# passcod/zarc

Hardware: AMD Instinct MI355X
Metric: uncompressed GiB/s (pack) at zstd -3 (higher is better)
Workload: dtype u8; 1 GPU; zarc pack 10000 x 1048576 B synthetic entries per GPU, zstd level 3, checksum on (BASELINE configs[1]); entries_per_gpu=10000, entries_total=10000, entry_bytes=1048576, level=3, kinds=text/records/lz/random round-robin

## Files before the change

zarc_amd/csrc/zarc_device.h:

```cpp
#pragma once
#include <hip/hip_runtime.h>
#include <stdint.h>

namespace zd {

constexpr int WAVE = 64;

__device__ __forceinline__ int lane_id() { return (int)(threadIdx.x & 63); }
__device__ __forceinline__ int wave_id() { return (int)(threadIdx.x >> 6); }

__device__ __forceinline__ void wave_sync()
{
#ifdef ZARC_HIPEMU
    hipemu_wave_sync();
#else
    __builtin_amdgcn_fence(__ATOMIC_RELEASE, "wavefront");
    __builtin_amdgcn_wave_barrier();
    __builtin_amdgcn_fence(__ATOMIC_ACQUIRE, "wavefront");
#endif
}

__device__ __forceinline__ void wave_lds_order()
{
#ifdef ZARC_HIPEMU
    hipemu_wave_sync();
#else
    asm volatile("" ::: "memory");
#endif
}

__device__ __forceinline__ void lds_barrier()
{
#ifdef ZARC_HIPEMU
    __syncthreads();
#else
    asm volatile("s_waitcnt lgkmcnt(0)\n\ts_barrier" ::: "memory");
#endif
}

template <int PRIO> __device__ __forceinline__ void wave_priority()
{
#ifndef ZARC_HIPEMU
    __builtin_amdgcn_s_setprio(PRIO);
#endif
}

__device__ __forceinline__ void wave_sync_global()
{
#ifdef ZARC_HIPEMU
    hipemu_wave_sync();
#else
    __builtin_amdgcn_fence(__ATOMIC_RELEASE, "workgroup");
    __builtin_amdgcn_wave_barrier();
    __builtin_amdgcn_fence(__ATOMIC_ACQUIRE, "workgroup");
#endif
}

__device__ __forceinline__ uint32_t uniform(uint32_t v)
{
#ifdef ZARC_HIPEMU
    return hipemu_readfirstlane(v);
#else
    return (uint32_t)__builtin_amdgcn_readfirstlane((int)v);
#endif
}

__device__ __forceinline__ uint32_t readlane(uint32_t v, uint32_t idx)
{
#ifdef ZARC_HIPEMU
    return hipemu_readfirstlane((uint32_t)__shfl((int)v, (int)idx, 64));
#else
    return (uint32_t)__builtin_amdgcn_readlane((int)v, (int)__builtin_amdgcn_readfirstlane((int)idx));
#endif
}

__device__ __forceinline__ uint64_t ballot(bool p) { return (uint64_t)__ballot(p ? 1 : 0); }
__device__ __forceinline__ uint32_t shfl(uint32_t v, int src) { return (uint32_t)__shfl((int)v, src, 64); }
__device__ __forceinline__ uint32_t shfl_up(uint32_t v, unsigned d) { return (uint32_t)__shfl_up((int)v, d, 64); }
__device__ __forceinline__ uint32_t shfl_down(uint32_t v, unsigned d) { return (uint32_t)__shfl_down((int)v, d, 64); }
__device__ __forceinline__ uint32_t shfl_xor(uint32_t v, int m) { return (uint32_t)__shfl_xor((int)v, m, 64); }

__device__ __forceinline__ uint32_t load_l2_u32(const uint32_t *p)
{
#ifdef ZARC_HIPEMU
    return *p;
#else
    return __hip_atomic_load(p, __ATOMIC_RELAXED, __HIP_MEMORY_SCOPE_AGENT);
#endif
}
__device__ __forceinline__ uint64_t load_l2_u64(const uint32_t *p)
{
#ifdef ZARC_HIPEMU
    return (uint64_t)p[0] | ((uint64_t)p[1] << 32);
#else
    return __hip_atomic_load((const uint64_t *)p, __ATOMIC_RELAXED, __HIP_MEMORY_SCOPE_AGENT);
#endif
}
__device__ __forceinline__ void atomic_max_l2(uint32_t *p, uint32_t v)
{
#ifdef ZARC_HIPEMU
    if (*p < v) *p = v;
#else
    (void)__hip_atomic_fetch_max(p, v, __ATOMIC_RELAXED, __HIP_MEMORY_SCOPE_AGENT);
#endif
}
__device__ __forceinline__ void wait_vmem()
{
#ifndef ZARC_HIPEMU
    asm volatile("s_waitcnt vmcnt(0)" ::: "memory");
#endif
}

__device__ __forceinline__ void store_streaming(uint64_t *p, uint64_t v)
{
#ifdef ZARC_HIPEMU
    *p = v;
#else
    __builtin_nontemporal_store(v, p);
#endif
}

__device__ __forceinline__ uint32_t rotr32(uint32_t x, int n) { return (x >> n) | (x << (32 - n)); }
__device__ __forceinline__ uint64_t rotl64(uint64_t x, int n) { return (x << n) | (x >> (64 - n)); }
__device__ __forceinline__ int hb32(uint32_t v) { return 31 - __clz((int)v); }
__device__ __forceinline__ int ctz64(uint64_t v) { return __ffsll((long long)v) - 1; }
__device__ __forceinline__ int ctz32(uint32_t v) { return __ffs((int)v) - 1; }

__device__ __forceinline__ uint32_t wave_scan_incl(uint32_t v)
{
#ifdef ZARC_HIPEMU
    int l = lane_id();
#pragma unroll
    for (int d = 1; d < 64; d <<= 1) {
        uint32_t t = shfl_up(v, (unsigned)d);
        if (l >= d) v += t;
    }
    return v;
#else
    v += (uint32_t)__builtin_amdgcn_update_dpp(0, (int)v, 0x111, 0xF, 0xF, false);
    v += (uint32_t)__builtin_amdgcn_update_dpp(0, (int)v, 0x112, 0xF, 0xF, false);
    v += (uint32_t)__builtin_amdgcn_update_dpp(0, (int)v, 0x114, 0xF, 0xF, false);
    v += (uint32_t)__builtin_amdgcn_update_dpp(0, (int)v, 0x118, 0xF, 0xF, false);
    v += (uint32_t)__builtin_amdgcn_update_dpp(0, (int)v, 0x142, 0xA, 0xF, false);
    v += (uint32_t)__builtin_amdgcn_update_dpp(0, (int)v, 0x143, 0xC, 0xF, false);
    return v;
#endif
}
__device__ __forceinline__ uint32_t shfl_up1(uint32_t v)
{
#ifdef ZARC_HIPEMU
    return shfl_up(v, 1u);
#else
    return (uint32_t)__builtin_amdgcn_update_dpp((int)v, (int)v, 0x138, 0xF, 0xF, false);
#endif
}
__device__ __forceinline__ uint32_t row_scan_incl(uint32_t v)
{
#ifdef ZARC_HIPEMU
    int l = lane_id() & 15;
#pragma unroll
    for (int d = 1; d < 16; d <<= 1) {
        uint32_t t = shfl_up(v, (unsigned)d);
        if (l >= d) v += t;
    }
    return v;
#else
    v += (uint32_t)__builtin_amdgcn_update_dpp(0, (int)v, 0x111, 0xF, 0xF, false);
    v += (uint32_t)__builtin_amdgcn_update_dpp(0, (int)v, 0x112, 0xF, 0xF, false);
    v += (uint32_t)__builtin_amdgcn_update_dpp(0, (int)v, 0x114, 0xF, 0xF, false);
    v += (uint32_t)__builtin_amdgcn_update_dpp(0, (int)v, 0x118, 0xF, 0xF, false);
    return v;
#endif
}
__device__ __forceinline__ uint32_t wave_sum(uint32_t v)
{
#pragma unroll
    for (int d = 32; d > 0; d >>= 1) v += shfl_xor(v, d);
    return v;
}
__device__ __forceinline__ uint32_t wave_max(uint32_t v)
{
#pragma unroll
    for (int d = 32; d > 0; d >>= 1) { uint32_t t = shfl_xor(v, d); v = t > v ? t : v; }
    return v;
}

__device__ __forceinline__ uint32_t load_u32(const uint8_t *p)
{
    uint32_t v;
    __builtin_memcpy(&v, p, 4);
    return v;
}
__device__ __forceinline__ uint64_t load_u64(const uint8_t *p)
{
    uint64_t v;
    __builtin_memcpy(&v, p, 8);
    return v;
}

}
```

zarc_amd/csrc/zge_match.hip:

```cpp
#include "zarc_device.h"
#include "zarc_kernels.h"

namespace {

#ifdef ZARC_HIPEMU
#define ZGE_CLOCK() 0ull
#else
#define ZGE_CLOCK() ((unsigned long long)__builtin_readcyclecounter())
#endif
#define ZGE_IDX(u) ((uint32_t)((wave * PER + (u)) * 64 + lane))
#ifndef ZGE_S2_DUPMASK
#define ZGE_S2_DUPMASK 0
#endif
#define ZGE_PROF(i) do { if ((dbg & 1024) && tid == 0) { const unsigned long long now_ = ZGE_CLOCK(); L.prof[i] += now_ - tprev; tprev = now_; } } while (0)

constexpr int TILE = 1024;
constexpr int THREADS = 512;
constexpr int WAVES = THREADS / 64;
constexpr int PER = TILE / THREADS;
static_assert(PER == 2, "the kernel is written for two positions per thread");
constexpr int CHUNKS = TILE / 64;
constexpr int TAG_BITS = 10;
constexpr uint32_t TAG_MASK = (1u << TAG_BITS) - 1;
struct U128 { uint64_t lo, hi; };
constexpr int CAP_MAX = 256;
constexpr int REP_BACK_MAX = 256;
constexpr int TB_BYTES = 12 + REP_BACK_MAX + TILE + CAP_MAX + 24;

template <int TAB_LOG, bool NEAR16> struct MatchLds {
    static constexpr int TAB_WORDS = NEAR16 ? (1 << TAB_LOG) / 2 : 2 << TAB_LOG;
    uint32_t tab[TAB_WORDS + (NEAR16 ? 1 : 0)];
    uint32_t a0[TILE], a1[TILE];
    uint32_t ex[TILE];
    uint32_t tb[2][(TB_BYTES + 3) / 4];
    uint32_t wcnt[CHUNKS];
    uint32_t wrep[2 * CHUNKS];
    uint32_t ctrl[16];
    unsigned long long prof[15];
};
enum { K_POS = 0, K_REP0 = 1, K_REP1 = 2, K_FLAG = 3, K_SLOT = 4, K_ANY = 5, K_CHG = 6 ,
       K_CEND = 10 ,
       K_CLEN = 11 ,
       K_LONG = 12 , K_LONG2 = 13  };

__device__ __forceinline__ uint32_t hash_long32(uint64_t v)
{
    const uint32_t lo = (uint32_t)v, hi = (uint32_t)(v >> 32);
    return lo * 0x9E3779B1u + hi * 0x85EBCA77u;
}
__device__ __forceinline__ uint32_t hash_far32(uint64_t v, uint32_t w) { return hash_long32(v) + w * 0xC2B2AE3Du; }
__device__ __forceinline__ uint32_t hash_short32(uint64_t v, int nbytes)
{
    uint32_t lo = (uint32_t)v, hi = (uint32_t)(v >> 32);
    if (nbytes < 8) hi &= (nbytes > 4) ? ((1u << (8 * (nbytes - 4))) - 1) : 0u;
    if (nbytes < 4) lo &= (1u << (8 * nbytes)) - 1;
    return lo * 0xC2B2AE3Du + hi * 0x27D4EB2Fu;
}

constexpr int REP_COST = 9;
constexpr int F_REP_BACK = 256, F_BACK_CAP = 8, F_LAZY_DELTA = 5, F_MIN_REP = 3, F_SEG_LOG = 21;
template <int MATCH_COST, int LITC> __device__ __forceinline__ int32_t score_mc(uint32_t len, uint32_t off, bool is_rep)
{
    static_assert(LITC == 5 || LITC == 6, "literal cost");
    const int32_t lits = (int32_t)((len << 2) + (LITC == 6 ? len << 1 : len));
    return is_rep ? lits - REP_COST : lits - MATCH_COST - zd::hb32(off);
}
#define score_of(P_, len_, off_, rep_) score_mc<MATCH_COST, LITC>((len_), (off_), (rep_))

template <bool WIDE> __device__ __forceinline__ uint32_t match_pack_w(uint32_t off, uint32_t len, bool rep) { return off | (len << 21) | ((rep ? 1u : 0u) << (WIDE ? 31 : 30)); }
__device__ __forceinline__ uint32_t match_off(uint32_t m) { return m & 0x1FFFFFu; }
template <bool WIDE> __device__ __forceinline__ uint32_t match_len_w(uint32_t m) { return (m >> 21) & (WIDE ? 0x3FFu : 0x1FFu); }
template <bool WIDE> __device__ __forceinline__ bool match_rep_w(uint32_t m) { return WIDE ? (m >> 31) != 0 : ((m >> 30) & 1u) != 0; }
#define match_pack(o_, l_, r_) match_pack_w<(CONT_CAP > 0 || EXT_ROUND)>((o_), (l_), (r_))
#define match_len(m_) match_len_w<(CONT_CAP > 0 || EXT_ROUND)>(m_)
#define match_rep(m_) match_rep_w<(CONT_CAP > 0 || EXT_ROUND)>(m_)
constexpr int LONG_CAP = 960;

__device__ __forceinline__ uint32_t wave_match_ext(const uint8_t *src, uint32_t p, uint32_t off, uint32_t from, uint32_t maxlen, int lane)
{
    static_assert(LONG_CAP <= 1024, "one trip of 64 x 16 bytes");
    const uint32_t at = from + 16u * (uint32_t)lane;
    const bool act = at < maxlen;
    U128 a{0, 0}, b{0, 0};
    if (act) { __builtin_memcpy(&a, src + (p + at), 16); __builtin_memcpy(&b, src + (p - off + at), 16); }
    const uint64_t xl = a.lo ^ b.lo, xh = a.hi ^ b.hi;
    const uint32_t mis = xl ? (uint32_t)(zd::ctz64(xl) >> 3) : (xh ? 8u + (uint32_t)(zd::ctz64(xh) >> 3) : 16u);
    const uint64_t bad = zd::ballot(act && mis < 16u);
    uint32_t len = maxlen;
    if (bad) {
        const uint32_t first = (uint32_t)zd::ctz64(bad);
        len = from + 16u * first + zd::readlane(mis, first);
        if (len > maxlen) len = maxlen;
    }
    return len;
}

struct StageWin { const uint32_t *w; int ndw; uint32_t wofs; };
static_assert((TB_BYTES + 3) / 4 <= THREADS, "one staged dword per thread");
__device__ __forceinline__ StageWin stage_window(const ZgeParams &P, const uint8_t *src, uint32_t n, uint32_t tile, uint32_t tend, uint32_t cap_max)
{
    (void)P;
    const uint32_t before = (uint32_t)F_REP_BACK + 8;
    const uint32_t lo = tile >= before ? tile - before : 0;
    uint32_t hi = tend + cap_max + 16;
    if (hi > n + 16) hi = n + 16;
    const uintptr_t a = (uintptr_t)(src + lo);
    const uint32_t mis = (uint32_t)(a & 3);
    StageWin s;
    s.w = (const uint32_t *)(a - mis);
    s.ndw = (int)((hi - lo + mis + 3) / 4);
    s.wofs = mis - lo;
    return s;
}

__device__ __forceinline__ uint32_t tile_end(uint32_t tile, uint32_t n)
{
    uint32_t e = tile + TILE;
    const uint32_t be = (tile / ZARC_BLOCK + 1) * ZARC_BLOCK;
    if (e > be) e = be;
    return e > n ? n : e;
}

}

template <int TAB_LOG, int SHORT_BYTES, int MATCH_COST, int F_FAR_LOG, int FAR_WAYS, bool FAR_SHORT, int FAR_STEP_LOG, int FAR_RES_LOG, int FAR_SKIP, int FAR_BACK, bool DIAG,
          bool NEAR16, int FAR_CDC, int LITC, int LAZY2, bool REP_PASS, int CONT_CAP, bool EXT_ROUND>
__device__ __forceinline__ void zge_match_body(MatchLds<TAB_LOG, NEAR16> &L, const ZgeParams &P, const uint8_t *__restrict__ src_base, const uint64_t *__restrict__ src_off,
                                               const uint64_t *__restrict__ src_len, const uint32_t *__restrict__ order, const uint32_t *__restrict__ units, uint32_t n_units,
                                               const uint64_t *__restrict__ block_prefix, ZgeBlock *__restrict__ blocks,
                                               uint64_t *__restrict__ seq_scratch, uint8_t *__restrict__ lit_scratch, uint32_t *__restrict__ queue,
                                               uint32_t *__restrict__ far_scratch)
{
    constexpr int NFAR = FAR_WAYS * (FAR_SHORT ? 2 : 1);
    constexpr int NTAB = 1 + NFAR;
    constexpr int far_shift = 32 - (F_FAR_LOG + TAG_BITS);
    constexpr uint32_t far_words = (uint32_t)(((size_t)FAR_WAYS << F_FAR_LOG) * (FAR_SHORT ? 2 : 1));
    uint32_t *const far_l = far_scratch + (size_t)blockIdx.x * far_words;
    uint32_t *const far_s = far_l + ((size_t)FAR_WAYS << F_FAR_LOG);
    constexpr uint32_t far_smask = (1u << FAR_STEP_LOG) - 1, far_rmask = (1u << FAR_RES_LOG) - 1;
    static_assert(FAR_BACK % 8 == 0 && FAR_BACK >= 8 && FAR_BACK <= 48, "backward extension of far candidates");
    static_assert(!FAR_CDC || (FAR_WAYS == 1 && !FAR_SHORT && far_shift >= FAR_CDC), "content-defined sampling: one way on the 12-byte hash");
    constexpr uint32_t cdc_mask = (1u << FAR_CDC) - 1;
    uint32_t *const Ltl = L.tab, *const Lts = L.tab + (NEAR16 ? 0 : (1 << TAB_LOG));
    typedef uint16_t __attribute__((may_alias)) u16a;
    u16a *const Lt16 = (u16a *)L.tab;
    const int tid = (int)threadIdx.x, lane = zd::lane_id();
    const uint32_t dbg = DIAG ? (uint32_t)P.dbg : 0u;
    const int wave = (int)zd::uniform((uint32_t)zd::wave_id());
    const uint64_t lt = (1ull << lane) - 1;
    const uint32_t seg_mask = (1u << F_SEG_LOG) - 1;
    const uint32_t cap_max = (uint32_t)(P.cap < CAP_MAX ? P.cap : CAP_MAX);
    unsigned long long tprev = ZGE_CLOCK();
    if (tid < 15) L.prof[tid] = 0;

    constexpr uint32_t SEG_BLOCKS = (1u << F_SEG_LOG) / ZARC_BLOCK;
    for (;;) {
    if (tid == 0) L.ctrl[K_SLOT] = atomicAdd(queue, 1u);
    zd::lds_barrier();
    const uint32_t unit = L.ctrl[K_SLOT];
    if (unit >= n_units) break;
    const uint32_t slot = units[2 * unit], ub0 = units[2 * unit + 1];
    const uint32_t f = order[slot];
    const uint8_t *src = src_base + src_off[f];
    const uint32_t n = (uint32_t)src_len[f];
    const uint32_t window = n <= (1u << P.window_log) ? (n ? n : 1u) : (1u << P.window_log);
    const uint32_t hash_end = n >= 8 ? n - 7 : 0;
    const bool far_on = NFAR && n > (uint32_t)P.far_min_frame;
    const uint32_t far_end = (far_on && n >= 12) ? n - 11 : 0;
    const uint64_t first_block = block_prefix[slot];
    const uint32_t nblocks = (uint32_t)(block_prefix[slot + 1] - first_block);

    for (int i = tid; i < MatchLds<TAB_LOG, NEAR16>::TAB_WORDS; i += THREADS) L.tab[i] = 0;
    if (NFAR && far_on) {
        uint4 *f4 = (uint4 *)far_l;
        for (uint32_t i = (uint32_t)tid; i < far_words / 4; i += THREADS) f4[i] = make_uint4(0, 0, 0, 0);
        zd::wait_vmem();
    }
    if (tid == 0) { L.ctrl[K_REP0] = 0; L.ctrl[K_REP1] = 0; }
    zd::lds_barrier();
    uint32_t cold = 0, skip_left = 0;
    constexpr bool FAR_COMPACT = FAR_RES_LOG > 0 && !FAR_CDC;
    constexpr int FNEXT_ROWS = FAR_COMPACT ? 1 : PER;
    uint32_t fnext[FNEXT_ROWS][NFAR ? NFAR : 1];
    uint32_t pf_far_tile = 0xFFFFFFFFu;
    uint32_t hfn[PER] = {0xFFFFFFFFu, 0xFFFFFFFFu};
    uint32_t pf_word = 0, pf_tile = 0xFFFFFFFFu;
    uint32_t lds_tile[2] = {0xFFFFFFFFu, 0xFFFFFFFFu};
#pragma unroll
    for (int u = 0; u < FNEXT_ROWS; u++)
#pragma unroll
        for (int k = 0; k < (NFAR ? NFAR : 1); k++) fnext[u][k] = 0;

    const uint32_t ub1 = (n > ZARC_SPLIT_MIN && ub0 + SEG_BLOCKS < nblocks) ? ub0 + SEG_BLOCKS : nblocks;
    for (uint32_t b = ub0; b < ub1; b++) {
        const uint32_t bs = b * ZARC_BLOCK;
        const uint32_t be = n - bs > ZARC_BLOCK ? bs + ZARC_BLOCK : n;
        const uint32_t blen = (uint32_t)(be - bs);
        ZgeBlock *rec = blocks + first_block + b;
        uint64_t *seq_out = seq_scratch + (first_block + b) * zge_seq_stride((uint32_t)P.slot_bytes);
        uint8_t *lit_out = lit_scratch + (first_block + b) * zge_lit_stride((uint32_t)P.slot_bytes);

        if (b > ub0 && (bs & seg_mask) == 0) {
            for (int i = tid; i < MatchLds<TAB_LOG, NEAR16>::TAB_WORDS; i += THREADS) L.tab[i] = 0;
            if (NFAR) {
                uint4 *f4 = (uint4 *)far_l;
                for (uint32_t i = (uint32_t)tid; i < far_words / 4; i += THREADS) f4[i] = make_uint4(0, 0, 0, 0);
                zd::wait_vmem();
                pf_far_tile = 0xFFFFFFFFu;
            }
        }
        if (tid == 0) { L.ctrl[K_FLAG] = 0; L.ctrl[K_POS] = 0; if (CONT_CAP) L.ctrl[K_CEND] = 0xFFFFFFFFu; }
        zd::lds_barrier();
        const uint8_t first = blen ? src[bs] : 0;
        const uint64_t pat = 0x0101010101010101ull * first;
        const uint64_t *w = (const uint64_t *)(src + bs);
        if (blen >= 1024 && tid < 128 && w[tid] != pat) L.ctrl[K_FLAG] = 1;
        zd::lds_barrier();
        if (L.ctrl[K_FLAG] == 0) {
            bool diff = false;
            const uint32_t nw = blen / 8;
            for (uint32_t i = (uint32_t)tid; i < nw; i += THREADS) diff |= w[i] != pat;
            for (uint32_t i = nw * 8 + (uint32_t)tid; i < blen; i += THREADS) diff |= src[bs + i] != first;
            if (diff) L.ctrl[K_FLAG] = 1;
        }
        zd::lds_barrier();
        const bool all_same = L.ctrl[K_FLAG] == 0;
        if (tid == 0) {
            rec->frame = f; rec->index = b; rec->src_len = blen; rec->nseq = 0; rec->nlit = 0;
            rec->type = (all_same && blen >= 2) ? 1u : 2u; rec->out_len = 0; rec->pad = 0;
        }
        if (all_same && blen >= 2) { zd::lds_barrier(); continue; }

        uint32_t nseq = 0, lp = 0;

        for (uint32_t tile = bs; tile < be; tile += TILE) {
            const uint32_t tend = be - tile > TILE ? tile + TILE : be;
            const uint32_t tcount = (uint32_t)(tend - tile);
            const uint32_t segbase = tile & ~seg_mask;
            zd::lds_barrier();
            ZGE_PROF(0);
            const uint32_t pos = bs + L.ctrl[K_POS];
            const bool cont = CONT_CAP && L.ctrl[K_CEND] == L.ctrl[K_POS] && pos >= tile;
            if (pos >= tend) { if (NFAR) zd::wait_vmem(); continue; }
            if (skip_left) {
                skip_left--;
                const uint32_t start = (uint32_t)((pos > tile ? pos : tile) - tile);
                {
                    const uint32_t cntb = tcount - start, k = (uint32_t)tid * 16;
                    const uint8_t *sp = src + tile + start;
                    uint8_t *dp = lit_out + lp;
                    if (!(dbg & 32)) {
                        if (k + 16 <= cntb) { U128 v; __builtin_memcpy(&v, sp + k, 16); __builtin_memcpy(dp + k, &v, 16); }
                        else for (uint32_t r = k; r < cntb; r++) dp[r] = sp[r];
                    }
                }
                lp += tcount - start;
                if (NFAR) zd::wait_vmem();
                zd::lds_barrier();
                if (tid == 0) L.ctrl[K_POS] = (uint32_t)(tend - bs);
                continue;
            }
            const uint32_t erep0 = L.ctrl[K_REP0], erep1 = L.ctrl[K_REP1];
            if (CONT_CAP && cont) {
                const uint32_t idx_c = pos - tile;
                if (wave == (int)(idx_c >> 7)) {
                    const uint32_t limit = (uint32_t)(be - pos);
                    uint32_t clen = 0;
                    if (erep0 != 0 && erep0 <= pos && erep0 <= window) clen = wave_match_ext(src, pos, erep0, 0, limit < (uint32_t)CONT_CAP ? limit : (uint32_t)CONT_CAP, lane);
                    if (lane == 0) L.ctrl[K_CLEN] = clen;
                }
            }
            if (tid == 0) L.ctrl[K_ANY] = 0;
            if (REP_PASS && tid < 4) L.ctrl[K_CHG + tid] = 0;
            if (EXT_ROUND && tid == 0) { L.ctrl[K_LONG] = 0; L.ctrl[K_LONG2] = 0; }

            const uint32_t bsel = (tile / TILE) & 1u;
            const uint8_t *const tbb = (const uint8_t *)L.tb[bsel];
            const uint8_t *const tbn = (const uint8_t *)L.tb[bsel ^ 1u];
            const StageWin sw = stage_window(P, src, n, tile, tend, cap_max);
            const uint32_t wofs = sw.wofs;
            const uint32_t ntile = tile + TILE;
            uint32_t wofs_n = 0;
            bool staged_now = false;
            {
                if (lds_tile[bsel] != tile) {
                    uint32_t v = pf_word;
                    if (pf_tile != tile && tid < sw.ndw) v = sw.w[tid];
                    if (tid < sw.ndw) L.tb[bsel][tid] = v;
                    lds_tile[bsel] = tile;
                    staged_now = true;
                }
                if (ntile < n) {
                    const StageWin nw = stage_window(P, src, n, ntile, tile_end(ntile, n), cap_max);
                    wofs_n = nw.wofs;
                    uint32_t v = pf_word;
                    if (pf_tile != ntile && tid < nw.ndw) v = nw.w[tid];
                    if (tid < nw.ndw) L.tb[bsel ^ 1u][tid] = v;
                    lds_tile[bsel ^ 1u] = ntile;
                    const uint32_t n2 = ntile + TILE;
                    if (n2 < n) {
                        const StageWin w2 = stage_window(P, src, n, n2, tile_end(n2, n), cap_max);
                        if (tid < w2.ndw) pf_word = w2.w[tid];
                        pf_tile = n2;
                    }
                }
            }
            if (staged_now) zd::lds_barrier();
            ZGE_PROF(1);
            uint64_t p8[PER];
            uint32_t fe[PER][NFAR ? NFAR : 1], ftag[PER][FAR_SHORT ? 2 : 1];
            uint32_t foffs[PER][NFAR ? NFAR : 1];
            uint64_t qf[PER][NFAR ? NFAR : 1];
            const bool far_ahead = NFAR && pf_far_tile == tile;
#pragma unroll
            for (int u = 0; u < PER; u++) {
                const uint32_t idx = ZGE_IDX(u);
                const uint32_t p = tile + idx;
                uint32_t hl = 0xFFFFFFFFu, hs = 0xFFFFFFFFu;
                p8[u] = 0;
#pragma unroll
                for (int k = 0; k < (NFAR ? NFAR : 1); k++) {
                    if (FAR_COMPACT) {
                        const uint32_t got = zd::shfl(fnext[0][k], (int)(((uint32_t)u * 64u + (uint32_t)lane) >> FAR_RES_LOG));
                        fe[u][k] = (far_ahead && !(idx & far_rmask)) ? got : 0u;
                    } else fe[u][k] = far_ahead ? fnext[FAR_COMPACT ? 0 : u][k] : 0u;
                    foffs[u][k] = 0; qf[u][k] = 0;
                }
                ftag[u][0] = 0xFFFFFFFFu;
                if (FAR_SHORT) ftag[u][1] = 0xFFFFFFFFu;
                uint32_t hfc = 0xFFFFFFFFu;
                if (idx < tcount) {
                    p8[u] = zd::load_u64(tbb + (uint32_t)(p + wofs));
                    if (p < hash_end && !(dbg & 64)) {
                        const uint32_t h32s = hash_short32(p8[u], SHORT_BYTES);
                        const uint32_t h32l = NEAR16 ? 0u : hash_long32(p8[u]);
                        hl = NEAR16 ? 0xFFFFFFFFu : h32l >> (32 - (TAB_LOG + TAG_BITS));
                        hs = NEAR16 ? h32s >> (32 - TAB_LOG) : h32s >> (32 - (TAB_LOG + TAG_BITS));
                        if (FAR_CDC) {
                            if (p < far_end && !(dbg & 2048)) {
                                if (far_ahead) hfc = hfn[u];
                                else {
                                    const uint32_t w8 = zd::load_u32(tbb + (uint32_t)(p + 8 + wofs));
                                    const uint32_t h32f = hash_far32(p8[u], w8);
                                    if (((h32f >> (far_shift - FAR_CDC)) & cdc_mask) == 0 && !((uint32_t)p8[u] == (uint32_t)(p8[u] >> 32) && (uint32_t)p8[u] == w8)) hfc = h32f >> far_shift;
                                }
                            }
                            if (hfc != 0xFFFFFFFFu) {
                                if (!far_ahead) fe[u][0] = zd::load_l2_u32(far_l + (size_t)(hfc >> TAG_BITS));
                                else {
                                    const uint32_t e = fe[u][0];
                                    uint32_t o = (e && (e & TAG_MASK) == (hfc & TAG_MASK) && !(dbg & 4096)) ? p - (segbase + (e >> TAG_BITS) - 1) : 0u;
                                    if (o + 8 > p || o > window || (dbg & 1)) o = 0;
                                    foffs[u][0] = o;
                                    if (o) qf[u][0] = zd::load_u64(src + (p - o));
                                }
                            }
                        } else
                        if (NFAR && p < far_end && !(p & far_rmask) && !(dbg & 2048)) {
                            const uint32_t hf = (h32l + zd::load_u32(tbb + (uint32_t)(p + 8 + wofs)) * 0xC2B2AE3Du) >> far_shift, hg = h32s >> far_shift;
                            ftag[u][0] = hf & TAG_MASK;
                            if (FAR_SHORT) ftag[u][1] = hg & TAG_MASK;
                            if (!far_ahead) {
                                if (FAR_WAYS == 2) {
                                    const uint64_t el = zd::load_l2_u64(far_l + (size_t)(hf >> TAG_BITS) * 2);
                                    fe[u][0] = (uint32_t)el; fe[u][1] = (uint32_t)(el >> 32);
                                    if (FAR_SHORT) { const uint64_t es = zd::load_l2_u64(far_s + (size_t)(hg >> TAG_BITS) * 2); fe[u][2] = (uint32_t)es; fe[u][3] = (uint32_t)(es >> 32); }
                                } else {
#pragma unroll
                                for (int w = 0; w < FAR_WAYS; w++) {
                                    fe[u][w] = zd::load_l2_u32(far_l + ((size_t)(hf >> TAG_BITS) * FAR_WAYS + w));
                                    if (FAR_SHORT) fe[u][FAR_WAYS + w] = zd::load_l2_u32(far_s + ((size_t)(hg >> TAG_BITS) * FAR_WAYS + w));
                                }
                                }
                            } else {
#pragma unroll
                                for (int k = 0; k < NFAR; k++) {
                                    const uint32_t e = fe[u][k];
                                    uint32_t o = (e && (e & TAG_MASK) == ftag[u][k / (FAR_WAYS ? FAR_WAYS : 1)] && !(dbg & 4096)) ? p - (segbase + (e >> TAG_BITS) - 1) : 0u;
#pragma unroll
                                    for (int j = 0; j < k; j++) if (o == foffs[u][j]) o = 0;
                                    if (o + 8 > p || o > window || (dbg & 1)) o = 0;
                                    foffs[u][k] = o;
                                    if (o) qf[u][k] = zd::load_u64(src + (p - o));
                                }
                            }
                        }
                    }
                }
                L.a0[idx] = NEAR16 ? (hs == 0xFFFFFFFFu ? (1u << TAB_LOG) : hs) : hl;
                if (!NEAR16) L.a1[idx] = hs;
                else if (FAR_CDC) L.a1[idx] = hfc;
                L.ex[idx] = 0;
            }
            zd::lds_barrier();
            ZGE_PROF(2);
            if (NEAR16) {
              if (wave == 0 && !(dbg & 4)) {
                zd::wave_priority<3>();
                uint32_t h[CHUNKS], e[CHUNKS];
#if ZGE_S2_DUPMASK
                uint64_t dupmask = 0;
#endif
#pragma unroll
                for (int k = 0; k < CHUNKS; k++) {
                    h[k] = L.a0[k * 64 + lane];
#if ZGE_S2_DUPMASK
                    const uint32_t hn = lane < 63 ? L.a0[k * 64 + lane + 1] : 0xFFFFFFFFu;
                    if (hn == h[k]) dupmask |= 1ull << k;
#endif
                }
#pragma unroll
                for (int k = 0; k < CHUNKS; k++) {
                    e[k] = (uint32_t)Lt16[h[k]];
                    zd::wave_lds_order();
#if ZGE_S2_DUPMASK
                    if (!((dupmask >> k) & 1))
#endif
                    Lt16[h[k]] = (uint16_t)((uint32_t)tile + (uint32_t)(k * 64 + lane));
                    zd::wave_lds_order();
                }
#pragma unroll
                for (int k = 0; k < CHUNKS; k++) L.a0[k * 64 + lane] = e[k];
                zd::wave_priority<0>();
              }
            } else
            if (wave < 2 && !(dbg & 4)) {
                zd::wave_priority<3>();
                uint32_t *tab = wave == 0 ? Ltl : Lts;
                uint32_t *hc = wave == 0 ? L.a0 : L.a1;
                uint32_t h[CHUNKS], e[CHUNKS];
                uint64_t dupmask = 0;
#pragma unroll
                for (int k = 0; k < CHUNKS; k++) {
                    h[k] = hc[k * 64 + lane];
                    const uint32_t hn = lane < 63 ? hc[k * 64 + lane + 1] : 0xFFFFFFFFu;
                    if (hn == h[k]) dupmask |= 1ull << k;
                }
#pragma unroll
                for (int k = 0; k < CHUNKS; k++) {
                    const bool act = h[k] != 0xFFFFFFFFu;
                    e[k] = act ? tab[h[k] >> TAG_BITS] : 0u;
                    zd::wave_lds_order();
                    if (act && !((dupmask >> k) & 1)) {
                        const uint32_t code = ((uint32_t)(tile - segbase) + (uint32_t)(k * 64 + lane) + 1) << TAG_BITS;
                        atomicMax(&tab[h[k] >> TAG_BITS], code | (h[k] & TAG_MASK));
                    }
                    zd::wave_lds_order();
                }
#pragma unroll
                for (int k = 0; k < CHUNKS; k++)
                    hc[k * 64 + lane] = e[k] ^ (h[k] & TAG_MASK);
                zd::wave_priority<0>();
            }
            if (NFAR) zd::wait_vmem();
            zd::lds_barrier();
            ZGE_PROF(3);
            uint32_t near_e[PER] = {0, 0};
            if (FAR_CDC) {
                uint64_t vnx[PER];
                uint32_t wnx[PER];
#pragma unroll
                for (int u = 0; u < PER; u++) {
                    const uint32_t pn = ntile + ZGE_IDX(u);
                    const uint32_t at = pn < far_end ? (uint32_t)(pn + wofs_n) : 0u;
                    vnx[u] = zd::load_u64(tbn + at);
                    wnx[u] = zd::load_u32(tbn + at + 8);
                    if (NEAR16) near_e[u] = L.a0[ZGE_IDX(u)];
                }
#pragma unroll
                for (int u = 0; u < PER; u++) {
                    const uint32_t pn = ntile + ZGE_IDX(u);
                    hfn[u] = 0xFFFFFFFFu;
                    fnext[u][0] = 0;
                    if (pn < far_end && !(dbg & (2048 | 32768))) {
                        const uint64_t vn = vnx[u];
                        const uint32_t wn = wnx[u];
                        const uint32_t h32f = hash_far32(vn, wn);
                        if (((h32f >> (far_shift - FAR_CDC)) & cdc_mask) == 0 && !((uint32_t)vn == (uint32_t)(vn >> 32) && (uint32_t)vn == wn)) {
                            hfn[u] = h32f >> far_shift;
                            fnext[u][0] = zd::load_l2_u32(far_l + (size_t)(hfn[u] >> TAG_BITS));
                        }
                    }
                }
                pf_far_tile = ntile;
            } else
            if (NFAR) {
#pragma unroll
                for (int u = 0; u < FNEXT_ROWS; u++) {
                    const uint32_t idxn = FAR_COMPACT ? (uint32_t)wave * 128u + ((uint32_t)lane << FAR_RES_LOG) : ZGE_IDX(u);
                    const uint32_t pn = ntile + idxn;
                    const bool mine = (!FAR_COMPACT || (uint32_t)lane < (128u >> FAR_RES_LOG)) && !((dbg & 16384) && wave < 2) && !(dbg & 32768);
                    if (mine && pn < far_end && !(pn & far_rmask) && !(dbg & 2048)) {
                        const uint64_t v = zd::load_u64(tbn + (uint32_t)(pn + wofs_n));
                        const uint32_t hf = hash_far32(v, zd::load_u32(tbn + (uint32_t)(pn + 8 + wofs_n))) >> far_shift, hg = hash_short32(v, SHORT_BYTES) >> far_shift;
                        if (FAR_WAYS == 2) {
                            const uint64_t el = zd::load_l2_u64(far_l + (size_t)(hf >> TAG_BITS) * 2);
                            fnext[u][0] = (uint32_t)el; fnext[u][1] = (uint32_t)(el >> 32);
                            if (FAR_SHORT) { const uint64_t es = zd::load_l2_u64(far_s + (size_t)(hg >> TAG_BITS) * 2); fnext[u][2] = (uint32_t)es; fnext[u][3] = (uint32_t)(es >> 32); }
                        } else {
#pragma unroll
                        for (int w = 0; w < FAR_WAYS; w++) {
                            fnext[u][w] = zd::load_l2_u32(far_l + ((size_t)(hf >> TAG_BITS) * FAR_WAYS + w));
                            if (FAR_SHORT) fnext[u][FAR_WAYS + w] = zd::load_l2_u32(far_s + ((size_t)(hg >> TAG_BITS) * FAR_WAYS + w));
                        }
                        }
                    } else {
#pragma unroll
                        for (int k = 0; k < NFAR; k++) fnext[u][k] = 0;
                    }
                }
                pf_far_tile = ntile;
            }
            uint32_t mo[PER], mw[PER];
            uint32_t offs[PER][NTAB];
            U128 q16[PER];
            bool fol[PER];
#pragma unroll
            for (int u = 0; u < PER; u++) {
                const uint32_t idx = ZGE_IDX(u);
                const uint32_t p = tile + idx;
                uint32_t cn = 0;
                fol[u] = false;
                if (NEAR16) {
                    const uint32_t d = ((p - (FAR_CDC ? near_e[u] : L.a0[idx]) - 1u) & 0xFFFFu) + 1u;
                    cn = (idx < tcount && p < hash_end && d <= p && !(dbg & (5 | 64))) ? p - d + 1 : 0u;
                } else
                if (idx < tcount && !(dbg & 5)) {
                    const uint32_t w0 = L.a0[idx], w1 = L.a1[idx];
                    const uint32_t wn = (w0 && !(w0 & TAG_MASK)) ? w0 : w1;
                    cn = (wn && !(wn & TAG_MASK)) ? segbase + (wn >> TAG_BITS) : 0u;
                }
                uint32_t on = cn ? p - (cn - 1) : 0u;
                if (on + 8 > p || on > window || idx >= tcount || (dbg & 1)) on = 0;
                offs[u][0] = on;
                if (NEAR16) { const uint32_t below = zd::shfl_up1(on); fol[u] = lane > 0 && on != 0 && on == below && !(dbg & 16); }
                q16[u] = U128{0, 0};
                if (on && !fol[u]) __builtin_memcpy(&q16[u], src + (p - on - 8), 16);
                if (NFAR && !far_ahead) {
#pragma unroll
                    for (int k = 0; k < NFAR; k++) {
                        const uint32_t e = fe[u][k];
                        const uint32_t want = FAR_CDC ? (L.a1[idx] == 0xFFFFFFFFu ? 0xFFFFFFFFu : (L.a1[idx] & TAG_MASK)) : ftag[u][k / (FAR_WAYS ? FAR_WAYS : 1)];
                        uint32_t o = (e && (e & TAG_MASK) == want && !(dbg & 4096)) ? p - (segbase + (e >> TAG_BITS) - 1) : 0u;
#pragma unroll
                        for (int j = 0; j < k; j++) if (o == foffs[u][j]) o = 0;
                        if (o + 8 > p || o > window || idx >= tcount || (dbg & 1)) o = 0;
                        foffs[u][k] = o;
                        if (o) qf[u][k] = zd::load_u64(src + (p - o));
                    }
                }
#pragma unroll
                for (int k = 0; k < NFAR; k++) offs[u][1 + k] = (foffs[u][k] == on && !fol[u]) ? 0u : foffs[u][k];
            }
            ZGE_PROF(9);
            uint32_t rres[PER];
            {
                const bool use0 = erep0 != 0 && erep0 <= window;
                const bool use1 = erep1 != 0 && erep1 != erep0 && erep1 <= window;
#pragma unroll
                for (int u = 0; u < PER; u++) {
                    const uint32_t idx = ZGE_IDX(u);
                    const uint32_t p = tile + idx;
                    const uint32_t limit = idx < tcount ? (uint32_t)(be - p) : 0u, cap = limit < cap_max ? limit : cap_max;
                    uint32_t res = 0;
#pragma unroll
                    for (int k = 0; k < 2; k++) {
                        const uint32_t off = k == 0 ? erep0 : erep1;
                        if (!(k == 0 ? use0 : use1) || off > idx + (uint32_t)F_REP_BACK || off > p || idx >= tcount || (dbg & 1)) continue;
                        uint64_t x = zd::load_u64(tbb + (uint32_t)(p - off + wofs)) ^ p8[u];
                        uint32_t len = 0;
                        while (!x && len + 8 < cap) {
                            const uint64_t a0 = zd::load_u64(tbb + (uint32_t)(p + len + 8 + wofs)), b0 = zd::load_u64(tbb + (uint32_t)(p - off + len + 8 + wofs));
                            const uint64_t a1 = zd::load_u64(tbb + (uint32_t)(p + len + 16 + wofs)), b1 = zd::load_u64(tbb + (uint32_t)(p - off + len + 16 + wofs));
                            len += 8;
                            x = a0 ^ b0;
                            if (!x && len + 8 < cap) { len += 8; x = a1 ^ b1; }
                        }
                        len += x ? (uint32_t)(zd::ctz64(x) >> 3) : 8u;
                        if (len > cap) len = cap;
                        if (len >= (uint32_t)F_MIN_REP && len > (res & 0x1FFu)) res = len | ((uint32_t)k << 9);
                    }
                    rres[u] = res;
                }
            }
            ZGE_PROF(10);
            auto prefix_len = [&](uint32_t p, uint64_t p8v, uint32_t cap, uint32_t off, uint64_t first8) -> uint32_t {
                uint64_t x = first8 ^ p8v;
                uint32_t len = 0;
                while (!x && len + 8 < cap) {
                    U128 sv;
                    __builtin_memcpy(&sv, src + (p - off + len + 8), 16);
                    const uint64_t a0 = zd::load_u64(tbb + (uint32_t)(p + len + 8 + wofs)), a1 = zd::load_u64(tbb + (uint32_t)(p + len + 16 + wofs));
                    len += 8;
                    x = a0 ^ sv.lo;
                    if (!x && len + 8 < cap) { len += 8; x = a1 ^ sv.hi; }
                }
                len += x ? (uint32_t)(zd::ctz64(x) >> 3) : 8u;
                return len > cap ? cap : len;
            };
            constexpr bool FAR_MERGED = NEAR16 && FAR_CDC && NFAR == 1;
            uint32_t b_len[PER], b_off[PER], b_flags[PER], near_acc[PER];
            int32_t b_score[PER];
#pragma unroll
            for (int u = 0; u < PER; u++) {
                const uint32_t idx = ZGE_IDX(u);
// ... 354 lines not shown
```

zarc_amd/csrc/zge_parse_round.h:

```cpp
#pragma unroll
            for (int u = 0; u < PER; u++) {
                const uint32_t idx = ZGE_IDX(u);
                const uint32_t len = mw[u] & 0xFFFF, back = (mw[u] >> 16) & 0xFF;
                if (len && back && !(dbg & 8)) {
                    const bool rep = (mw[u] >> 24) & 1;
                    const int32_t base = score_of(P, len, mo[u], rep);
                    const uint32_t lim = back < idx ? back : idx;
#pragma unroll
                    for (uint32_t k = 1; k <= (uint32_t)F_BACK_CAP; k++) {
                        const int32_t sc = base + LITC * (int32_t)k;
                        if (k <= lim && sc > 0) atomicMax(&L.ex[idx - k], ((uint32_t)sc << 6) | (63u - k));
                    }
                    for (uint32_t k = (uint32_t)F_BACK_CAP + 1; k <= lim; k++) {
                        const int32_t sc = base + LITC * (int32_t)k;
                        if (sc > 0) atomicMax(&L.ex[idx - k], ((uint32_t)sc << 6) | (63u - k));
                    }
                }
            }
#if ZGE_FIRST
                ZGE_PROF(12);
                if (NFAR) zd::wait_vmem();
                ZGE_PROF(13);
#endif
            zd::lds_barrier();
#if ZGE_FIRST
            ZGE_PROF(4);
            if (NFAR) {
                const uint32_t way = (tile / TILE) & (uint32_t)(FAR_WAYS - 1);
#pragma unroll
                for (int u = 0; u < PER; u++) {
                    const uint32_t idx = ZGE_IDX(u);
                    const uint32_t p = tile + idx;
                    if (FAR_CDC) {
                        const uint32_t hfc = L.a1[idx];
                        if (hfc != 0xFFFFFFFFu && !(dbg & (64 | 8192)))
                            zd::atomic_max_l2(far_l + (size_t)(hfc >> TAG_BITS), ((((uint32_t)(tile - segbase) + idx + 1) << TAG_BITS)) | (hfc & TAG_MASK));
                    } else
                    if (idx < tcount && p < far_end && (p & far_smask) <= far_rmask && !(dbg & (64 | 8192))) {
                        const uint32_t code = ((uint32_t)(tile - segbase) + idx + 1) << TAG_BITS;
                        const uint32_t hf = hash_far32(p8[u], zd::load_u32(tbb + (uint32_t)(p + 8 + wofs))) >> far_shift;
                        zd::atomic_max_l2(far_l + ((size_t)(hf >> TAG_BITS) * FAR_WAYS + way), code | (hf & TAG_MASK));
                        if (FAR_SHORT) {
                            const uint32_t hg = hash_short32(p8[u], SHORT_BYTES) >> far_shift;
                            zd::atomic_max_l2(far_s + ((size_t)(hg >> TAG_BITS) * FAR_WAYS + way), code | (hg & TAG_MASK));
                        }
                    }
                }
            }
            if (L.ctrl[K_ANY] == 0) {
                const uint32_t start = (uint32_t)((pos > tile ? pos : tile) - tile);
#pragma unroll
                for (int u = 0; u < PER; u++) {
                    const uint32_t idx = ZGE_IDX(u);
                    if (idx >= start && idx < tcount && !(dbg & 32)) lit_out[lp + (idx - start)] = (uint8_t)p8[u];
                }
                lp += tcount - start;
                if (tid == 0) { L.ctrl[K_POS] = (uint32_t)(tend - bs); if (CONT_CAP) L.ctrl[K_CEND] = 0xFFFFFFFFu; }
                cold++;
                if (cold >= 2) skip_left = cold >= 4 ? 7u : (1u << (cold - 1)) - 1;
                if (NFAR) zd::wait_vmem();
                continue;
            }
            cold = 0;
#endif
#pragma unroll
            for (int u = 0; u < PER; u++) {
                const uint32_t idx = ZGE_IDX(u);
                const uint32_t offer = L.ex[idx];
                uint32_t blen_ = mw[u] & 0xFFFF, boff = mo[u];
                bool brep = (mw[u] >> 24) & 1;
                if (offer) {
                    const int32_t own = blen_ ? score_of(P, blen_, boff, brep) : 0;
                    if ((int32_t)(offer >> 6) > own) {
                        const uint32_t k = 63u - (offer & 63u);
                        const uint32_t nm = L.a0[idx + k];
                        boff = match_off(nm);
                        blen_ = match_len(nm) + k;
                        brep = match_rep(nm);
                    }
                }
                fo[u] = boff;
                fw[u] = blen_ | ((brep ? 1u : 0u) << 24);
                L.a1[idx] = match_pack(boff, blen_, brep);
            }
            zd::lds_barrier();
            ZGE_PROF(5);
            bool take[PER];
            uint32_t nx[PER];
#pragma unroll
            for (int u = 0; u < PER; u++) {
                const uint32_t idx = ZGE_IDX(u);
                const uint32_t my_len = fw[u] & 0xFFFF;
                take[u] = idx < tcount && my_len != 0;
                if (take[u] && P.lazy && idx + 1 < tcount) {
                    const uint32_t m2 = L.a1[idx + 1];
                    const uint32_t l2 = match_len(m2);
                    if (l2 && score_of(P, l2, match_off(m2), match_rep(m2)) > score_of(P, my_len, fo[u], (fw[u] >> 24) & 1) + F_LAZY_DELTA) take[u] = false;
                }
                if (LAZY2 && take[u] && idx + 2 < tcount) {
                    const uint32_t m3 = L.a1[idx + 2];
                    const uint32_t l3 = match_len(m3);
                    if (l3 && score_of(P, l3, match_off(m3), match_rep(m3)) > score_of(P, my_len, fo[u], (fw[u] >> 24) & 1) + LAZY2) take[u] = false;
                }
                nx[u] = take[u] ? idx + my_len : idx + 1;
            }
            {
                uint32_t val[PER];
#pragma unroll
                for (int u = 0; u < PER; u++) {
                    const uint32_t cbase = (uint32_t)(wave * PER + u) * 64;
                    const uint32_t cend = cbase + 64 < tcount ? cbase + 64 : tcount;
                    val[u] = nx[u];
#pragma unroll
                    for (int r = 0; r < 6; r++) {
                        const uint32_t v2 = zd::shfl(val[u], (int)((val[u] - cbase) & 63));
                        if (val[u] < cend) val[u] = v2;
                    }
                }
                {
                    const uint32_t obase = (uint32_t)(wave * PER + 1) * 64, oend = obase + 64 < tcount ? obase + 64 : tcount;
                    const uint32_t through = zd::shfl(val[1], (int)((val[0] - obase) & 63));
                    if (val[0] >= obase && val[0] < oend) val[0] = through;
                }
#pragma unroll
                for (int u = 0; u < PER; u++) L.ex[ZGE_IDX(u)] = val[u];
            }
            zd::lds_barrier();
            ZGE_PROF(6);
            {
                zd::wave_priority<2>();
                uint32_t cur = (uint32_t)((pos > tile ? pos : tile) - tile);
                int c = 0;
#pragma unroll
                for (; c < wave; c++) {
                    const uint32_t pend = (uint32_t)(c * 128 + 128) < tcount ? (uint32_t)(c * 128 + 128) : tcount;
                    if (cur < pend) cur = L.ex[cur];
                }
                cur = zd::uniform(cur);
#pragma unroll
                for (int u = 0; u < PER; u++) {
                    const int mychunk = wave * PER + u;
                    const uint32_t cbase = (uint32_t)mychunk * 64;
                    const uint32_t cend = cbase + 64 < tcount ? cbase + 64 : tcount;
                    const uint64_t tk = zd::ballot(take[u]);
                    const uint32_t span = cend > cbase ? cend - cbase : 0u;
                    uint64_t sel = 0, lits = 0;
                    const uint32_t entry = cur;
                    uint32_t o_last = 0, o_diff = 0;
                    if (!(dbg & 2)) {
                        while (cur < cend) {
                            const uint64_t ahead = tk & (~0ull << (cur - cbase));
                            if (ahead == 0) { cur = cend; break; }
                            const uint32_t q = (uint32_t)zd::ctz64(ahead);
                            sel |= 1ull << q;
                            cur = zd::readlane(nx[u], q);
                            if (REP_PASS) { const uint32_t o = zd::readlane(fo[u], q); if (o != o_last) { o_diff = o_last; o_last = o; } }
                        }
                        const uint64_t below = sel & lt;
                        const uint32_t qs = below ? 63u - (uint32_t)__clzll((long long)below) : 0u;
                        const uint32_t over = zd::shfl(nx[u], (int)qs);
                        const uint32_t me = cbase + (uint32_t)lane;
                        lits = zd::ballot(me >= entry && (uint32_t)lane < span && !((sel >> lane) & 1) && (!below || over <= me));
                    }
                    msel[u] = sel;
                    mlit[u] = lits;
                    if (lane == 0) L.wcnt[mychunk] = ((uint32_t)__popcll(msel[u]) << 16) | (uint32_t)__popcll(mlit[u]);
                    if (REP_PASS && lane == 0) { L.wrep[2 * mychunk] = o_last; L.wrep[2 * mychunk + 1] = o_diff; }
                }
                if (wave == WAVES - 1 && lane == 0) L.ctrl[K_POS] = (uint32_t)(tile - bs) + cur;
                zd::wave_priority<0>();
            }
            zd::lds_barrier();
            ZGE_PROF(7);
```

Before: 42.67 GiB/s.

## Replace short-range backward LDS atomicMax offers with DPP cross-lane max propagation

The backward-extension offers over the first F_BACK_CAP positions are now built in registers with a DPP shift-down max chain across the two per-thread positions. Only the wave-boundary spill is written to LDS with atomicMax, and each position takes the larger of its register offer and the LDS value. This is meant to remove most of the per-position LDS atomicMax traffic in the parse round. The diff also moves the hash table to the end of the LDS struct and replaces typed pointer loads with byte-pointer memcpy loads, which mainly affects alignment handling. The key encoding changes slightly: the sc>0 check is dropped and the low bits now come from a precomputed KEY_STEP term, so correctness relies on that encoding matching.

Measured after the change: 43.04 GiB/s (median of 6 runs). No clear change (+0.9%).

```diff
diff --git a/zarc_amd/csrc/zarc_device.h b/zarc_amd/csrc/zarc_device.h
--- a/zarc_amd/csrc/zarc_device.h
+++ b/zarc_amd/csrc/zarc_device.h
@@ -154,6 +154,40 @@
     return (uint32_t)__builtin_amdgcn_update_dpp((int)v, (int)v, 0x138, 0xF, 0xF, false);
 #endif
 }
+__device__ __forceinline__ uint32_t shfl_down1_fill(uint32_t v, uint32_t fill)
+{
+#ifdef ZARC_HIPEMU
+    const uint32_t t = shfl_down(v, 1u);
+    return lane_id() == 63 ? fill : t;
+#else
+    return (uint32_t)__builtin_amdgcn_update_dpp((int)fill, (int)v, 0x130, 0xF, 0xF, false);
+#endif
+}
+__device__ __forceinline__ uint32_t shfl_down1_zero(uint32_t v)
+{
+#ifdef ZARC_HIPEMU
+    return shfl_down1_fill(v, 0u);
+#else
+    return (uint32_t)__builtin_amdgcn_update_dpp(0, (int)v, 0x130, 0xF, 0xF, true);
+#endif
+}
+__device__ __forceinline__ uint32_t shfl_up1_fill(uint32_t v, uint32_t fill)
+{
+#ifdef ZARC_HIPEMU
+    const uint32_t t = shfl_up(v, 1u);
+    return lane_id() == 0 ? fill : t;
+#else
+    return (uint32_t)__builtin_amdgcn_update_dpp((int)fill, (int)v, 0x138, 0xF, 0xF, false);
+#endif
+}
+__device__ __forceinline__ uint32_t rot_down1(uint32_t v)
+{
+#ifdef ZARC_HIPEMU
+    return shfl(v, (lane_id() + 1) & 63);
+#else
+    return (uint32_t)__builtin_amdgcn_update_dpp((int)v, (int)v, 0x134, 0xF, 0xF, false);
+#endif
+}
 __device__ __forceinline__ uint32_t row_scan_incl(uint32_t v)
 {
 #ifdef ZARC_HIPEMU
diff --git a/zarc_amd/csrc/zge_match.hip b/zarc_amd/csrc/zge_match.hip
--- a/zarc_amd/csrc/zge_match.hip
+++ b/zarc_amd/csrc/zge_match.hip
@@ -29,7 +29,6 @@
 
 template <int TAB_LOG, bool NEAR16> struct MatchLds {
     static constexpr int TAB_WORDS = NEAR16 ? (1 << TAB_LOG) / 2 : 2 << TAB_LOG;
-    uint32_t tab[TAB_WORDS + (NEAR16 ? 1 : 0)];
     uint32_t a0[TILE], a1[TILE];
     uint32_t ex[TILE];
     uint32_t tb[2][(TB_BYTES + 3) / 4];
@@ -37,6 +36,7 @@
     uint32_t wrep[2 * CHUNKS];
     uint32_t ctrl[16];
     unsigned long long prof[15];
+    uint32_t tab[TAB_WORDS + (NEAR16 ? 1 : 0)];
 };
 enum { K_POS = 0, K_REP0 = 1, K_REP1 = 2, K_FLAG = 3, K_SLOT = 4, K_ANY = 5, K_CHG = 6 ,
        K_CEND = 10 ,
@@ -95,7 +95,7 @@
     return len;
 }
 
-struct StageWin { const uint32_t *w; int ndw; uint32_t wofs; };
+struct StageWin { const uint8_t *w; int ndw; uint32_t wofs; };
 static_assert((TB_BYTES + 3) / 4 <= THREADS, "one staged dword per thread");
 __device__ __forceinline__ StageWin stage_window(const ZgeParams &P, const uint8_t *src, uint32_t n, uint32_t tile, uint32_t tend, uint32_t cap_max)
 {
@@ -107,7 +107,7 @@
     const uintptr_t a = (uintptr_t)(src + lo);
     const uint32_t mis = (uint32_t)(a & 3);
     StageWin s;
-    s.w = (const uint32_t *)(a - mis);
+    s.w = (const uint8_t *)(a - mis);
     s.ndw = (int)((hi - lo + mis + 3) / 4);
     s.wofs = mis - lo;
     return s;
@@ -141,6 +141,7 @@
     static_assert(FAR_BACK % 8 == 0 && FAR_BACK >= 8 && FAR_BACK <= 48, "backward extension of far candidates");
     static_assert(!FAR_CDC || (FAR_WAYS == 1 && !FAR_SHORT && far_shift >= FAR_CDC), "content-defined sampling: one way on the 12-byte hash");
     constexpr uint32_t cdc_mask = (1u << FAR_CDC) - 1;
+    constexpr uint32_t KEY_STEP = ((uint32_t)LITC << 6) - 1u;
     uint32_t *const Ltl = L.tab, *const Lts = L.tab + (NEAR16 ? 0 : (1 << TAB_LOG));
     typedef uint16_t __attribute__((may_alias)) u16a;
     u16a *const Lt16 = (u16a *)L.tab;
@@ -172,8 +173,7 @@
 
     for (int i = tid; i < MatchLds<TAB_LOG, NEAR16>::TAB_WORDS; i += THREADS) L.tab[i] = 0;
     if (NFAR && far_on) {
-        uint4 *f4 = (uint4 *)far_l;
-        for (uint32_t i = (uint32_t)tid; i < far_words / 4; i += THREADS) f4[i] = make_uint4(0, 0, 0, 0);
+        for (uint32_t i = (uint32_t)tid; i < far_words / 4; i += THREADS) *(uint4 *)((uint8_t *)far_l + 16u * i) = make_uint4(0, 0, 0, 0);
         zd::wait_vmem();
     }
     if (tid == 0) { L.ctrl[K_REP0] = 0; L.ctrl[K_REP1] = 0; }
@@ -203,8 +203,7 @@
         if (b > ub0 && (bs & seg_mask) == 0) {
             for (int i = tid; i < MatchLds<TAB_LOG, NEAR16>::TAB_WORDS; i += THREADS) L.tab[i] = 0;
             if (NFAR) {
-                uint4 *f4 = (uint4 *)far_l;
-                for (uint32_t i = (uint32_t)tid; i < far_words / 4; i += THREADS) f4[i] = make_uint4(0, 0, 0, 0);
+                for (uint32_t i = (uint32_t)tid; i < far_words / 4; i += THREADS) *(uint4 *)((uint8_t *)far_l + 16u * i) = make_uint4(0, 0, 0, 0);
                 zd::wait_vmem();
                 pf_far_tile = 0xFFFFFFFFu;
             }
@@ -213,13 +212,13 @@
         zd::lds_barrier();
         const uint8_t first = blen ? src[bs] : 0;
         const uint64_t pat = 0x0101010101010101ull * first;
-        const uint64_t *w = (const uint64_t *)(src + bs);
-        if (blen >= 1024 && tid < 128 && w[tid] != pat) L.ctrl[K_FLAG] = 1;
+        const uint8_t *w = src + bs;
+        if (blen >= 1024 && tid < 128 && zd::load_u64(w + 8u * (uint32_t)tid) != pat) L.ctrl[K_FLAG] = 1;
         zd::lds_barrier();
         if (L.ctrl[K_FLAG] == 0) {
             bool diff = false;
             const uint32_t nw = blen / 8;
-            for (uint32_t i = (uint32_t)tid; i < nw; i += THREADS) diff |= w[i] != pat;
+            for (uint32_t i = (uint32_t)tid; i < nw; i += THREADS) diff |= zd::load_u64(w + 8u * i) != pat;
             for (uint32_t i = nw * 8 + (uint32_t)tid; i < blen; i += THREADS) diff |= src[bs + i] != first;
             if (diff) L.ctrl[K_FLAG] = 1;
         }
@@ -285,7 +284,7 @@
             {
                 if (lds_tile[bsel] != tile) {
                     uint32_t v = pf_word;
-                    if (pf_tile != tile && tid < sw.ndw) v = sw.w[tid];
+                    if (pf_tile != tile && tid < sw.ndw) v = zd::load_u32(sw.w + 4u * (uint32_t)tid);
                     if (tid < sw.ndw) L.tb[bsel][tid] = v;
                     lds_tile[bsel] = tile;
                     staged_now = true;
@@ -294,13 +293,13 @@
                     const StageWin nw = stage_window(P, src, n, ntile, tile_end(ntile, n), cap_max);
                     wofs_n = nw.wofs;
                     uint32_t v = pf_word;
-                    if (pf_tile != ntile && tid < nw.ndw) v = nw.w[tid];
+                    if (pf_tile != ntile && tid < nw.ndw) v = zd::load_u32(nw.w + 4u * (uint32_t)tid);
                     if (tid < nw.ndw) L.tb[bsel ^ 1u][tid] = v;
                     lds_tile[bsel ^ 1u] = ntile;
                     const uint32_t n2 = ntile + TILE;
                     if (n2 < n) {
                         const StageWin w2 = stage_window(P, src, n, n2, tile_end(n2, n), cap_max);
-                        if (tid < w2.ndw) pf_word = w2.w[tid];
+                        if (tid < w2.ndw) pf_word = zd::load_u32(w2.w + 4u * (uint32_t)tid);
                         pf_tile = n2;
                     }
                 }
diff --git a/zarc_amd/csrc/zge_parse_round.h b/zarc_amd/csrc/zge_parse_round.h
--- a/zarc_amd/csrc/zge_parse_round.h
+++ b/zarc_amd/csrc/zge_parse_round.h
@@ -1,21 +1,32 @@
+            uint32_t roffer[PER];
+            {
+                uint32_t key0[PER], lim[PER];
 #pragma unroll
-            for (int u = 0; u < PER; u++) {
-                const uint32_t idx = ZGE_IDX(u);
-                const uint32_t len = mw[u] & 0xFFFF, back = (mw[u] >> 16) & 0xFF;
-                if (len && back && !(dbg & 8)) {
-                    const bool rep = (mw[u] >> 24) & 1;
-                    const int32_t base = score_of(P, len, mo[u], rep);
-                    const uint32_t lim = back < idx ? back : idx;
+                for (int u = 0; u < PER; u++) {
+                    const uint32_t idx = ZGE_IDX(u);
+                    const uint32_t len = mw[u] & 0xFFFF, back = (mw[u] >> 16) & 0xFF;
+                    const int32_t base = score_of(P, len, mo[u], (mw[u] >> 24) & 1);
+                    key0[u] = ((uint32_t)base << 6) | 63u;
+                    lim[u] = (len && !(dbg & 8)) ? (back < idx ? back : idx) : 0u;
+                    if (NFAR && FAR_BACK > F_BACK_CAP)
+                        for (uint32_t k = (uint32_t)F_BACK_CAP + 1; k <= lim[u]; k++) atomicMax(&L.ex[idx - k], key0[u] + k * KEY_STEP);
+                }
+                uint32_t acc[PER] = {0, 0}, edge = 0;
 #pragma unroll
-                    for (uint32_t k = 1; k <= (uint32_t)F_BACK_CAP; k++) {
-                        const int32_t sc = base + LITC * (int32_t)k;
-                        if (k <= lim && sc > 0) atomicMax(&L.ex[idx - k], ((uint32_t)sc << 6) | (63u - k));
+                for (uint32_t k = (uint32_t)F_BACK_CAP; k >= 1; k--) {
+                    uint32_t from0 = 0, from1 = 0;
+                    if (k < (uint32_t)F_BACK_CAP) {
+                        from1 = zd::shfl_down1_zero(acc[1]);
+                        from0 = zd::shfl_down1_fill(acc[0], zd::rot_down1(acc[1]));
                     }
-                    for (uint32_t k = (uint32_t)F_BACK_CAP + 1; k <= lim; k++) {
-                        const int32_t sc = base + LITC * (int32_t)k;
-                        if (sc > 0) atomicMax(&L.ex[idx - k], ((uint32_t)sc << 6) | (63u - k));
-                    }
+                    const uint32_t v0 = k <= lim[0] ? key0[0] + k * KEY_STEP : 0u, v1 = k <= lim[1] ? key0[1] + k * KEY_STEP : 0u;
+                    acc[0] = v0 > from0 ? v0 : from0;
+                    acc[1] = v1 > from1 ? v1 : from1;
+                    edge = zd::shfl_up1_fill(edge, acc[0]);
                 }
+                roffer[0] = zd::shfl_down1_fill(acc[0], zd::rot_down1(acc[1]));
+                roffer[1] = zd::shfl_down1_zero(acc[1]);
+                if (wave > 0 && lane < F_BACK_CAP && edge) atomicMax(&L.ex[(uint32_t)(wave * PER * 64 - 1 - lane)], edge);
             }
 #if ZGE_FIRST
                 ZGE_PROF(12);
@@ -66,7 +77,8 @@
 #pragma unroll
             for (int u = 0; u < PER; u++) {
                 const uint32_t idx = ZGE_IDX(u);
-                const uint32_t offer = L.ex[idx];
+                const uint32_t far_offer = L.ex[idx];
+                const uint32_t offer = roffer[u] > far_offer ? roffer[u] : far_offer;
                 uint32_t blen_ = mw[u] & 0xFFFF, boff = mo[u];
                 bool brep = (mw[u] >> 24) & 1;
                 if (offer) {
```
